# denix56/SI-Mamba

Measured on AMD Instinct MI355X. Metric: point-clouds/sec (fwd+bwd), higher is better.
Workload: dtype f32; 1 GPU; PointMamba classifier train step (FPS+kNN grouping, encoder, spectral SAST ordering, 12 Mamba blocks d=384 at L=1024, head, AdamW), 1024 pts -> 128 patches; global_batch=64, per_gpu_batch=64, npoints=1024, patches=128, mamba_seq_len=1024, parallelism=dp1, communicator_ranks=1, library_gemm=tuned solution table (si_mamba_amd/tuned/gemm_gfx950.csv)

## Files before the change

### include/simamba.h

```cpp
#ifndef SIMAMBA_H_
#define SIMAMBA_H_

#include <stddef.h>

#ifdef __cplusplus
extern "C" {
#endif

#define SIMAMBA_ABI_VERSION 9

#define SIMAMBA_F32  0
#define SIMAMBA_BF16 1

#define SIMAMBA_OK            0
#define SIMAMBA_E_NULLPTR    -1
#define SIMAMBA_E_SHAPE      -2
#define SIMAMBA_E_DTYPE      -3
#define SIMAMBA_E_DSTATE     -4
#define SIMAMBA_E_WIDTH      -5
#define SIMAMBA_E_WORKSPACE  -6
#define SIMAMBA_E_GROUPS     -7
#define SIMAMBA_E_ALIGN      -8
#define SIMAMBA_E_VARIANT    -9
#define SIMAMBA_E_BIAS       -10
// ... 107 lines not shown
                               int dim, int hidden_dtype, int out_dtype, void* stream);

#define SIMAMBA_NORM_RMS 1
int simamba_add_layer_norm_fwd_ex(const void* hidden, const float* residual, const float* rowscale,
                                  const float* weight, const float* bias, float* residual_out,
                                  void* normed, float* mean, float* rstd, int batch, int rows_per_batch,
                                  int dim, float eps, int hidden_dtype, int out_dtype, int flags, void* stream);
int simamba_add_layer_norm_bwd_ex(const void* dnormed, const float* dresidual_out,
                                  const float* residual_out, const float* mean, const float* rstd,
                                  const float* weight, const float* rowscale, float* dresidual,
                                  void* dhidden, float* dwb_partial, int batch, int rows_per_batch,
                                  int dim, int hidden_dtype, int out_dtype, int flags, void* stream);

int simamba_out_proj_add_ln_fwd(const void* y, const void* w, const float* residual, const float* rowscale,
                                const float* gamma, const float* beta, float* residual_out, void* normed, float* mean,
                                float* rstd, int batch, int K, int L, int C, float eps, int out_dtype, void* stream);
int simamba_out_proj_add_ln_fwd_ex(const void* y, const void* w, const float* residual, const float* rowscale,
                                   const float* gamma, const float* beta, float* residual_out, void* normed,
                                   float* mean, float* rstd, int batch, int K, int L, int C, float eps, int out_dtype,
                                   int flags, void* stream);

int simamba_in_proj_fwd(const void* x, const void* w, void* xz, int batch, int L, int C, int M, int io_dtype,
                        void* stream);

int simamba_bn_relu_grid(long long rows);
int simamba_bn_relu_fwd(const void* x, const float* gterm, int group, const float* weight, const float* bias,
                        float* running_mean, float* running_var, float momentum, float eps, int training,
                        void* y, float* mean, float* invstd, float* partial, long long rows, int C,
                        long long ld, int io_dtype, void* stream);
int simamba_bn_relu_bwd(const void* dy, const void* x, const float* gterm, int group, const float* weight,
                        const float* bias, const float* mean, const float* invstd, void* dx, float* dgterm,
                        int dgroup, float* dweight, float* dbias, float* partial, long long rows, int C,
                        long long ld, int io_dtype, int training, void* stream);
int simamba_bn_stats_local(const void* x, const float* gterm, int group, double* stats, long long stats_ld,
                           float* partial, long long rows, int C, long long ld, int io_dtype, void* stream);
int simamba_bn_stats_merge(const double* stats, int world, float* running_mean, float* running_var, float momentum,
                           float eps, float* mean, float* invstd, double* count, int C, void* stream);
int simamba_bn_relu_apply(const void* x, const float* gterm, int group, const float* weight, const float* bias,
                          const float* mean, const float* invstd, void* y, long long rows, int C, long long ld,
                          int io_dtype, void* stream);
int simamba_bn_relu_bwd_sums(const void* dy, const void* x, const float* gterm, int group, const float* weight,
                             const float* bias, const float* mean, const float* invstd, float* dweight,
                             float* dbias, float* partial, long long rows, int C, long long ld, int io_dtype,
                             void* stream);
int simamba_bn_relu_bwd_dx(const void* dy, const void* x, const float* gterm, int group, const float* weight,
                           const float* bias, const float* mean, const float* invstd, const float* sum_dweight,
                           const float* sum_dbias, const double* count, void* dx, float* dgterm, int dgroup,
                           long long rows, int C, long long ld, int io_dtype, void* stream);
int simamba_group_max_fwd(const void* x, void* out, unsigned char* idx, long long groups, int n, int C,
                          int io_dtype, void* stream);
int simamba_group_max_bwd(const void* dout, const unsigned char* idx, void* dx, long long groups, int n, int C,
                          int io_dtype, void* stream);

int simamba_three_nn(const float* xyz1, const float* xyz2, int* idx, float* weight, int batch, int N, int S,
                     void* stream);
int simamba_three_interpolate_fwd(const void* feats, const int* idx, const float* weight, void* out, int batch,
                                  int N, int S, int C, int io_dtype, void* stream);
int simamba_three_interpolate_bwd(const void* dout, const int* idx, const float* weight, float* dfeats, int batch,
                                  int N, int S, int C, int io_dtype, void* stream);

int simamba_chamfer_fwd(const float* pred, const float* gt, float* dist, unsigned char* idx1, unsigned char* idx2,
                        long long pairs, int n, int m, void* stream);
int simamba_chamfer_bwd(const float* pred, const float* gt, const float* ddist, const unsigned char* idx1,
                        const unsigned char* idx2, float* dpred, long long pairs, int n, int m, void* stream);

int simamba_knn_group(const float* points, const float* centers, long long* idx, int batch, int N, int G, int K,
                      void* stream);
int simamba_knn_group_ex(const float* points, const float* centers, const long long* len_points,
                         const long long* len_centers, long long* idx, int batch, int N, int G, int K, void* stream);

#define SIMAMBA_SPEC_SYMMETRIC   0x01u
#define SIMAMBA_SPEC_SELF_LOOP   0x02u
#define SIMAMBA_SPEC_BINARY      0x04u
#define SIMAMBA_SPEC_MATRIX_SYM  0x08u
#define SIMAMBA_SPEC_SMALLEST    0x10u
#define SIMAMBA_SPEC_SIGMA_MEAN  0x20u
#define SIMAMBA_SPEC_LARGE_G     0x40u

int simamba_knn_graph(const float* points, float* adj, void* workspace, size_t ws_bytes,
                      int B, int G, int F, int knn, float alpha, unsigned flags, void* stream);

int simamba_laplacian_topk(const float* adj, float* evals, float* evecs, long long* order,
                           float* all_evals, float* all_evecs, int B, int G, int k,
                           unsigned flags, void* stream);

size_t simamba_laplacian_topk_workspace_bytes(int B, int G);
int simamba_laplacian_topk_ex(const float* adj, float* evals, float* evecs, long long* order,
                              void* workspace, size_t ws_bytes, int B, int G, int k, unsigned flags,
                              void* stream);

size_t simamba_spectral_workspace_bytes(int B, int G);

int simamba_spectral_topk(const float* centers, float* evals, float* evecs, long long* order,
                          void* workspace, size_t ws_bytes, int B, int G, int knn, float alpha,
                          int k, unsigned flags, void* stream);

int simamba_farthest_point_sample(const float* points, long long* idx, float* centers, int B, int N,
                                  int K, void* stream);
int simamba_farthest_point_sample_ex(const float* points, const long long* lengths, const long long* start,
                                     long long* idx, float* centers, int B, int N, int K, void* stream);

int simamba_argsort_rows(const float* vals, long long* idx, int rows, int n, void* stream);

#ifdef __cplusplus
}
#endif
// ... 2 lines not shown
```

### si_mamba_amd/_lib.py

```python
from __future__ import annotations

import ctypes
import os
from ctypes import c_char_p, c_float, c_int, c_longlong, c_size_t, c_uint, c_void_p

_HERE = os.path.dirname(os.path.abspath(__file__))
LIB_PATH = os.path.join(_HERE, "libsimamba_hip.so")

F32, BF16 = 0, 1

SPEC_SYMMETRIC = 0x01
SPEC_SELF_LOOP = 0x02
SPEC_BINARY = 0x04
SPEC_MATRIX_SYM = 0x08
SPEC_SMALLEST = 0x10
SPEC_SIGMA_MEAN = 0x20
SPEC_LARGE_G = 0x40
SPEC_MAX_G = 128
SPEC_MAX_G_LARGE = 512

SCAN_AUTO, SCAN_ROWSCAN, SCAN_LPC2, SCAN_LPC4, SCAN_MIX = 0, 1, 2, 4, 6
CKPT_ROW, CKPT_SEQ = 128, 16
BWD_DETERMINISTIC = 1
NORM_RMS = 1
# ... 21 lines not shown
    "simamba_selective_scan_bwd_ex": (c_int, [_P, _P, _P, _P, _P, _P, _P, _P, _P, _P,
                                              _P, _P, _P, _P, _P, _P, _P, _P,
                                              c_int, c_int, c_int, c_int, c_int, c_int,
                                              _LL, _LL, _LL, _LL, _LL, c_int, c_int, _P, _LL, _P]),
    "simamba_selective_scan_dt_fwd": (c_int, [_P, _P, _P, _P, _P, _P, _P, _P, _P, _P,
                                              c_int, c_int, c_int, c_int, c_int, c_int,
                                              _LL, _LL, _LL, c_int, c_int, _P]),
    "simamba_selective_scan_dt_bwd": (c_int, [_P, _P, _P, _P, _P, _P, _P, _P, _P,
                                              _P, _P, _P, _P, _P, _P, _P, _P,
                                              c_int, c_int, c_int, c_int, c_int, c_int,
                                              _LL, _LL, _LL, _LL, _P]),
    "simamba_selective_scan_dt_bwd_ex": (c_int, [_P, _P, _P, _P, _P, _P, _P, _P, _P,
                                                 _P, _P, _P, _P, _P, _P, _P, _P,
                                                 c_int, c_int, c_int, c_int, c_int, c_int,
                                                 _LL, _LL, _LL, _LL, c_int, _P, _LL, _P]),
    "simamba_xdt_proj_fwd": (c_int, [_P, _P, _P, _P, _P, c_int, c_int, c_int, c_int, c_int, c_int, _LL, _P]),
    "simamba_conv_xdt_proj_fwd": (c_int, [_P, _P, _P, _P, _P, _P, _P, _P, c_int, c_int, c_int, c_int, c_int, c_int, _LL,
                                          _P]),
    "simamba_seq_gather_fwd": (c_int, [_P, _P, _P, c_int, c_int, c_int, c_int, _LL, c_int, _P]),
    "simamba_seq_gather_bwd": (c_int, [_P, _P, _P, c_int, c_int, c_int, c_int, c_int, _LL, c_int, _P]),
    "simamba_causal_conv1d_fwd": (c_int, [_P, _P, _P, _P, c_int, c_int, c_int, c_int, c_int, c_int, _LL, _P]),
    "simamba_causal_conv1d_bwd": (c_int, [_P, _P, _P, _P, _P, _P, _P,
                                          c_int, c_int, c_int, c_int, c_int, c_int, _LL, _LL, _P]),
    "simamba_causal_conv1d_bwd_workspace_floats": (_LL, [c_int, c_int, c_int, c_int, c_int]),
    "simamba_causal_conv1d_bwd_ex": (c_int, [_P, _P, _P, _P, _P, _P, _P,
                                             c_int, c_int, c_int, c_int, c_int, c_int, _LL, _LL, c_int, _P, _LL, _P]),
    "simamba_add_layer_norm_grid": (c_int, [c_int, c_int]),
    "simamba_add_layer_norm_fwd": (c_int, [_P, _P, _P, _P, _P, _P, _P, _P, _P, c_int, c_int, c_int, c_float,
                                           c_int, c_int, _P]),
    "simamba_add_layer_norm_bwd": (c_int, [_P, _P, _P, _P, _P, _P, _P, _P, _P, _P, c_int, c_int, c_int,
                                           c_int, c_int, _P]),
    "simamba_add_layer_norm_fwd_ex": (c_int, [_P, _P, _P, _P, _P, _P, _P, _P, _P, c_int, c_int, c_int, c_float,
                                              c_int, c_int, c_int, _P]),
    "simamba_add_layer_norm_bwd_ex": (c_int, [_P, _P, _P, _P, _P, _P, _P, _P, _P, _P, c_int, c_int, c_int,
                                              c_int, c_int, c_int, _P]),
    "simamba_out_proj_add_ln_fwd": (c_int, [_P, _P, _P, _P, _P, _P, _P, _P, _P, _P, c_int, c_int, c_int, c_int, c_float,
                                            c_int, _P]),
    "simamba_out_proj_add_ln_fwd_ex": (c_int, [_P, _P, _P, _P, _P, _P, _P, _P, _P, _P, c_int, c_int, c_int, c_int,
                                               c_float, c_int, c_int, _P]),
    "simamba_in_proj_fwd": (c_int, [_P, _P, _P, c_int, c_int, c_int, c_int, c_int, _P]),
    "simamba_bn_relu_grid": (c_int, [_LL]),
    "simamba_bn_relu_fwd": (c_int, [_P, _P, c_int, _P, _P, _P, _P, c_float, c_float, c_int, _P, _P, _P, _P, _LL, c_int,
                                    _LL, c_int, _P]),
    "simamba_bn_relu_bwd": (c_int, [_P, _P, _P, c_int, _P, _P, _P, _P, _P, _P, c_int, _P, _P, _P, _LL, c_int, _LL,
                                    c_int, c_int, _P]),
    "simamba_bn_stats_local": (c_int, [_P, _P, c_int, _P, _LL, _P, _LL, c_int, _LL, c_int, _P]),
    "simamba_bn_stats_merge": (c_int, [_P, c_int, _P, _P, c_float, c_float, _P, _P, _P, c_int, _P]),
    "simamba_bn_relu_apply": (c_int, [_P, _P, c_int, _P, _P, _P, _P, _P, _LL, c_int, _LL, c_int, _P]),
    "simamba_bn_relu_bwd_sums": (c_int, [_P, _P, _P, c_int, _P, _P, _P, _P, _P, _P, _P, _LL, c_int, _LL, c_int, _P]),
    "simamba_bn_relu_bwd_dx": (c_int, [_P, _P, _P, c_int, _P, _P, _P, _P, _P, _P, _P, _P, _P, c_int, _LL, c_int, _LL,
                                       c_int, _P]),
    "simamba_group_max_fwd": (c_int, [_P, _P, _P, _LL, c_int, c_int, c_int, _P]),
    "simamba_group_max_bwd": (c_int, [_P, _P, _P, _LL, c_int, c_int, c_int, _P]),
    "simamba_three_nn": (c_int, [_P, _P, _P, _P, c_int, c_int, c_int, _P]),
    "simamba_three_interpolate_fwd": (c_int, [_P, _P, _P, _P, c_int, c_int, c_int, c_int, c_int, _P]),
    "simamba_three_interpolate_bwd": (c_int, [_P, _P, _P, _P, c_int, c_int, c_int, c_int, c_int, _P]),
    "simamba_chamfer_fwd": (c_int, [_P, _P, _P, _P, _P, _LL, c_int, c_int, _P]),
    "simamba_chamfer_bwd": (c_int, [_P, _P, _P, _P, _P, _P, _LL, c_int, c_int, _P]),
    "simamba_knn_group": (c_int, [_P, _P, _P, c_int, c_int, c_int, c_int, _P]),
    "simamba_knn_group_ex": (c_int, [_P, _P, _P, _P, _P, c_int, c_int, c_int, c_int, _P]),
    "simamba_knn_graph": (c_int, [_P, _P, _P, c_size_t, c_int, c_int, c_int, c_int, c_float, c_uint, _P]),
    "simamba_laplacian_topk": (c_int, [_P, _P, _P, _P, _P, _P, c_int, c_int, c_int, c_uint, _P]),
    "simamba_laplacian_topk_workspace_bytes": (c_size_t, [c_int, c_int]),
    "simamba_laplacian_topk_ex": (c_int, [_P, _P, _P, _P, _P, c_size_t, c_int, c_int, c_int, c_uint, _P]),
    "simamba_spectral_workspace_bytes": (c_size_t, [c_int, c_int]),
    "simamba_spectral_topk": (c_int, [_P, _P, _P, _P, _P, c_size_t, c_int, c_int, c_int, c_float,
                                      c_int, c_uint, _P]),
    "simamba_argsort_rows": (c_int, [_P, _P, c_int, c_int, _P]),
    "simamba_farthest_point_sample": (c_int, [_P, _P, _P, c_int, c_int, c_int, _P]),
    "simamba_farthest_point_sample_ex": (c_int, [_P, _P, _P, _P, _P, c_int, c_int, c_int, _P]),
}

_lib = None


def load():
    global _lib
    if _lib is not None:
        return _lib
    if not os.path.exists(LIB_PATH):
        raise RuntimeError(
            f"{LIB_PATH} not found: build it with `python -c 'import __graft_entry__ as g; g.build()'` "
            "or `make -C si_mamba_amd/csrc`.  si_mamba_amd has no CPU / eager fallback.")
    lib = ctypes.CDLL(LIB_PATH)
    for name, (res, args) in SIGNATURES.items():
        fn = getattr(lib, name)
        fn.restype = res
        fn.argtypes = args
    got = lib.simamba_abi_version()
    if got != ABI_VERSION:
        raise RuntimeError(f"libsimamba_hip.so ABI version {got}, binding expects {ABI_VERSION}")
    _lib = lib
    return lib


def check(rc: int, what: str):
    if rc != 0:
        msg = load().simamba_strerror(rc).decode()
        raise RuntimeError(f"{what} failed (rc={rc}): {msg}")


def ptr(t):
    return None if t is None else t.data_ptr()


def dtype_code(dtype):
# ... 81 lines not shown

class scan_variant(_Override):
    cell, coerce = _scan_variant, int

    def __init__(self, variant):
        super().__init__(variant)


def current_scan_variant():
    return _scan_variant[0]


_scan_ckpt = [0]


class scan_ckpt(_Override):
    cell, coerce = _scan_ckpt, int

    def __init__(self, step):
        super().__init__(step)


_spectral_large_g = [False]


class spectral_large_g(_Override):
    cell = _spectral_large_g

    def __init__(self, on=True):
        super().__init__(on)


def spectral_large_g_forced():
    return _spectral_large_g[0]


_fuse_dt = [None]
counters = {}


def count(name):
    counters[name] = counters.get(name, 0) + 1


class scan_fuse_dt(_Override):
    cell, coerce = _fuse_dt, staticmethod(_tristate)


def fuse_dt_enabled(dtype):
    import torch
    return (dtype == torch.bfloat16) if _fuse_dt[0] is None else _fuse_dt[0]


_fuse_out_norm = [True]
_hand_in_proj = [None]


class fuse_out_norm(_Override):
    cell = _fuse_out_norm


def fuse_out_norm_enabled():
    return _fuse_out_norm[0]


class hand_in_proj(_Override):
    cell, coerce = _hand_in_proj, staticmethod(_tristate)


def in_proj_hand_enabled(workgroups, dtype=None):
    import torch
    if _hand_in_proj[0] is not None:
        return _hand_in_proj[0]
    return dtype != torch.float32 and workgroups >= IN_PROJ_MIN_WORKGROUPS


IN_PROJ_MIN_WORKGROUPS = 192


def scan_plan_step(batch, dim, seqlen, dstate, dtype, *, softplus=True, has_z=True, act_addr_or=0, a_addr=0,
                   b_addr=0, c_addr=0, z_bs=0, dz_bs=0, bc_strides=(0, 0, 0)):
    lib = load()
    code = dtype_code(dtype)
    step = _scan_ckpt[0] or lib.simamba_scan_ckpt_step(batch, dim, seqlen, dstate, code)
    if step == CKPT_SEQ and not lib.simamba_scan_seq_applicable(
            batch, dim, seqlen, dstate, code, int(bool(softplus)), int(bool(has_z)), act_addr_or, a_addr, b_addr,
            c_addr, z_bs, dz_bs, *bc_strides):
        step = CKPT_ROW
    if _scan_variant[0] == SCAN_ROWSCAN:
        step = CKPT_ROW
    return step


def mixer_scan_operands(xz_addr, a_addr, dim, seqlen, dt_rank, dstate, esz, xz_bs):
    S = dt_rank + 2 * dstate
    return dict(softplus=True, has_z=True, act_addr_or=xz_addr | (xz_addr + dim * seqlen * esz), a_addr=a_addr,
                b_addr=dt_rank * esz, c_addr=(dt_rank + dstate) * esz, z_bs=xz_bs, dz_bs=xz_bs,
                bc_strides=(seqlen * S, 1, S))


def scan_plan(batch, dim, seqlen, dstate, dtype, device, need_grad, **operands):
    import torch
    step = scan_plan_step(batch, dim, seqlen, dstate, dtype, **operands)
    count("scan_ckpt_seq" if step == CKPT_SEQ else "scan_ckpt_row")
    if not need_grad:
        return step, None
# ... 46 lines not shown
```

### si_mamba_amd/encoder_ops.py

```python
from __future__ import annotations

import torch
import torch.distributed as dist

from . import _lib


_BN_MAX_C = 1024
_BN_CHUNK = 256


_SPLITK = 64
_SPLITK_MIN_ROWS = 512


class TokenLinearFn(torch.autograd.Function):

    @staticmethod
    def forward(ctx, x, weight, bias):
        y = torch.nn.functional.linear(x, weight, bias)
        ctx.save_for_backward(x, weight)
        ctx.has_bias = bias is not None
        return y

    @staticmethod
    def backward(ctx, dy):
        x, weight = ctx.saved_tensors
        dy = dy.contiguous()
        io = dy.dtype
        rows, n_out = dy.shape
        dx = dw = db = None
        if ctx.needs_input_grad[0]:
            dx = (dy @ weight.to(io)).to(x.dtype)
        if ctx.needs_input_grad[1]:
            xc = x.to(io).contiguous()
            if rows % _SPLITK == 0 and rows // _SPLITK >= _SPLITK_MIN_ROWS:
                m = rows // _SPLITK
                a = dy.view(_SPLITK, m, n_out).transpose(1, 2)
                b = xc.view(_SPLITK, m, xc.shape[1])
                part = torch.bmm(a, b) if io == torch.float32 else torch.bmm(a, b, out_dtype=torch.float32)
                dw = part.sum(0).to(weight.dtype)
            else:
                dw = (dy.t() @ xc).to(weight.dtype)
        if ctx.has_bias and ctx.needs_input_grad[2]:
            db = dy.sum(0, dtype=torch.float32).to(weight.dtype)
        return dx, dw, db


def token_linear(x, weight, bias=None):
    if x.is_cuda and x.dim() == 2 and torch.is_grad_enabled() and (weight.requires_grad or x.requires_grad):
        return TokenLinearFn.apply(x, weight, bias)
    return torch.nn.functional.linear(x, weight, bias)


def _slices(C):
    return [(c0, min(c0 + _BN_MAX_C, C)) for c0 in range(0, C, _BN_MAX_C)]


def _off(t, elems):
    return None if t is None else t.data_ptr() + elems * t.element_size()


def _abi(name, *args):
    _lib.check(getattr(_lib.load(), name)(*args), name)


def _slice_of(g, c0, c1, C):
    return None if g is None else (g if (c0 == 0 and c1 == C) else g[:, c0:c1].contiguous())


def _bn_partial(lib, rows, C, dev):
    return torch.empty(lib.simamba_bn_relu_grid(rows), 2, min(C, _BN_MAX_C), device=dev, dtype=torch.float32)


def _bn_operands(x, gterm, weight, bias):
    xc = x.contiguous()
    g, w, b = (None if t is None else t.float().contiguous() for t in (gterm, weight, bias))
    mean = torch.empty(xc.shape[1], device=xc.device, dtype=torch.float32)
    return xc, g, w, b, torch.empty_like(xc), mean, torch.empty_like(mean)


def _dtypes(*tensors):
    return tuple(None if t is None else t.dtype for t in tensors)


def _bn_grads(dtypes, dx, dgt, dw, db):
    xdtype, gdtype, wdtype, bdtype = dtypes
    return (dx.to(xdtype), None if dgt is None else dgt.to(gdtype), None,
            None if wdtype is None else dw.to(wdtype), None if bdtype is None else db.to(bdtype),
            None, None, None, None, None)


def _bn_dgroup(g, group):
    dgroup = 0 if g is None else (group if _BN_CHUNK % group == 0 else _BN_CHUNK)
    if g is not None and dgroup == _BN_CHUNK and group % _BN_CHUNK != 0:
        raise ValueError("bn_relu_fn: group must divide 256 or be a multiple of it")
    return dgroup


# ... 148 lines not shown
def _bn_step(bn):
    training = bn.training or bn.running_mean is None
    momentum = bn.momentum
    if bn.training and bn.track_running_stats and bn.num_batches_tracked is not None:
        bn.num_batches_tracked.add_(1)
        if momentum is None:
            momentum = 1.0 / float(bn.num_batches_tracked)
    rm = bn.running_mean if (bn.track_running_stats and (bn.training or not training)) else None
    rv = bn.running_var if rm is not None else None
    return training, 0.0 if momentum is None else momentum, rm, rv


def _dist_up():
    return dist.is_available() and dist.is_initialized()


def _bn_relu_local(x, bn, gterm, group):
    training, momentum, rm, rv = _bn_step(bn)
    return BnReluFn.apply(x, gterm, group, bn.weight, bn.bias, rm, rv, momentum, bn.eps, training)


def sync_bn_relu_fn(x, bn, gterm=None, group=0, process_group=None):
    if not isinstance(bn, (torch.nn.BatchNorm1d, torch.nn.SyncBatchNorm)):
        raise TypeError(f"sync_bn_relu_fn: expected nn.SyncBatchNorm or nn.BatchNorm1d, got {type(bn).__name__}")
    if not bn.training:
        return _bn_relu_local(x, bn, gterm, group)
    if x.shape[0] < 1:
        raise ValueError(f"sync_bn_relu_fn: this rank holds {x.shape[0]} rows; every rank needs at least 1")
    if not _dist_up():
        raise RuntimeError("sync_bn_relu_fn: torch.distributed has no initialised process group")
    if x.is_cuda and torch.cuda.is_current_stream_capturing():
        raise RuntimeError(_CAPTURE_MSG)
    if process_group is None:
        process_group = getattr(bn, "process_group", None)
    _, momentum, rm, rv = _bn_step(bn)
    return SyncBnReluFn.apply(x, gterm, group, bn.weight, bn.bias, rm, rv, momentum, bn.eps, process_group)


def _sync_world(bn):
    return dist.get_world_size(bn.process_group) if _dist_up() else 1


def bn_relu_fn(x, bn: torch.nn.BatchNorm1d, gterm=None, group=0):
    if type(bn) is torch.nn.SyncBatchNorm:
        if bn.training and _sync_world(bn) > 1:
            return sync_bn_relu_fn(x, bn, gterm=gterm, group=group)
    elif type(bn) is not torch.nn.BatchNorm1d:
        if gterm is not None:
            x = x + gterm.to(x.dtype).repeat_interleave(group, dim=0)
        return torch.relu(bn(x))
    return _bn_relu_local(x, bn, gterm, group)


class GroupMaxFn(torch.autograd.Function):
    @staticmethod
    def forward(ctx, x):
        _lib.require_gpu(x, "group_max_fn")
        xc = x.contiguous()
        groups, n, C = xc.shape
        dev = xc.device
        code = _lib.dtype_code(xc.dtype)
        out = torch.empty(groups, C, device=dev, dtype=xc.dtype)
        idx = torch.empty(groups, C, device=dev, dtype=torch.uint8)
        with torch.cuda.device(dev):
            _abi("simamba_group_max_fwd", xc.data_ptr(), out.data_ptr(), idx.data_ptr(), groups, n, C, code,
                 _lib.stream_ptr(dev))
        ctx.save_for_backward(idx)
        ctx.meta = (groups, n, C, code, xc.dtype)
        return out

    @staticmethod
    def backward(ctx, dout):
        (idx,) = ctx.saved_tensors
        groups, n, C, code, dtype = ctx.meta
        d = dout.to(dtype).contiguous()
        dx = torch.empty(groups, n, C, device=d.device, dtype=dtype)
        with torch.cuda.device(d.device):
            _abi("simamba_group_max_bwd", d.data_ptr(), idx.data_ptr(), dx.data_ptr(), groups, n, C, code,
                 _lib.stream_ptr(d.device))
        return dx


def group_max_fn(x):
    return GroupMaxFn.apply(x)
```

### si_mamba_amd/point_mamba.py

```python
from __future__ import annotations

from types import SimpleNamespace

import torch
import torch.nn as nn

from . import grouping, spectral
from .block import MixerModel
from .add_norm import add_layer_norm_fn
from .encoder_ops import bn_relu_fn, group_max_fn, token_linear


class Group(nn.Module):

    def __init__(self, num_group, group_size):
        super().__init__()
        self.num_group = num_group
        self.group_size = group_size
        self.fps_fn = grouping.sample_farthest_points

    @torch.no_grad()
    def _indices(self, xyz, lengths=None):
        if lengths is not None:
            if not (xyz.is_cuda and xyz.shape[1] <= 8192):
                raise NotImplementedError("Group: lengths are taken by the HIP kernels only (a ROCm device, clouds of "
                                          "up to 8192 points)")
            need = max(self.num_group, self.group_size)
            if not torch.cuda.is_current_stream_capturing():
                shortest = int(lengths.min())
                if shortest < need:
                    raise ValueError(f"Group: the shortest cloud has {shortest} points, every cloud needs at least "
                                     f"{need} (max of num_group = {self.num_group} and group_size = {self.group_size})")
            center, _ = self.fps_fn(xyz, self.num_group, lengths=lengths)
            return center, grouping.knn_group(center, xyz, self.group_size, lengths=lengths)
        center, _ = self.fps_fn(xyz, self.num_group)
        if xyz.is_cuda and xyz.shape[1] <= 8192:
            return center, grouping.knn_group(center, xyz, self.group_size)
        d = torch.cdist(center, xyz)
        nn_idx = d.topk(self.group_size, dim=-1, largest=False, sorted=False)[1]
        return center, nn_idx

    def forward(self, xyz, *, lengths=None):
        B, N, _ = xyz.shape
        center, nn_idx = self._indices(xyz, lengths)
        flat = (nn_idx + torch.arange(B, device=xyz.device).view(-1, 1, 1) * N).view(-1)
        nb = xyz.reshape(B * N, -1)[flat].view(B, self.num_group, self.group_size, 3).contiguous()
        return nb - center.unsqueeze(2), center, nb


class Encoder(nn.Module):

    def __init__(self, encoder_channel):
        super().__init__()
        self.encoder_channel = encoder_channel
        self.fused = True
        self.first_conv = nn.Sequential(nn.Conv1d(3, 128, 1), nn.BatchNorm1d(128), nn.ReLU(inplace=True),
                                        nn.Conv1d(128, 256, 1))
        self.second_conv = nn.Sequential(nn.Conv1d(512, 512, 1), nn.BatchNorm1d(512), nn.ReLU(inplace=True),
                                         nn.Conv1d(512, self.encoder_channel, 1))

    def forward(self, point_groups):
        bs, g, n, _ = point_groups.shape
        c1, bn1, _, c2 = self.first_conv
        c3, bn2, _, c4 = self.second_conv
        lin = torch.nn.functional.linear
        x = point_groups.reshape(bs * g * n, 3)
        if self.fused and x.is_cuda and 256 % n == 0:
            lin = token_linear
            x = bn_relu_fn(lin(x, c1.weight.squeeze(-1), c1.bias), bn1)
            f = lin(x, c2.weight.squeeze(-1), c2.bias)
            cf = f.shape[1]
            fg = group_max_fn(f.view(bs * g, n, cf))
            w3 = c3.weight.squeeze(-1)
            gterm = lin(fg, w3[:, :cf], c3.bias)
            x = bn_relu_fn(lin(f, w3[:, cf:]), bn2, gterm=gterm, group=n)
            f = lin(x, c4.weight.squeeze(-1), c4.bias)
            return group_max_fn(f.view(bs * g, n, self.encoder_channel)).reshape(bs, g, self.encoder_channel)
        x = torch.relu(bn1(lin(x, c1.weight.squeeze(-1), c1.bias)))
        f = lin(x, c2.weight.squeeze(-1), c2.bias).view(bs * g, n, 256)
        fg = f.max(dim=1, keepdim=True)[0]
        x = torch.cat([fg.expand(-1, n, -1), f], dim=2).reshape(bs * g * n, 512)
        x = torch.relu(bn2(lin(x, c3.weight.squeeze(-1), c3.bias)))
        f = lin(x, c4.weight.squeeze(-1), c4.bias).view(bs * g, n, self.encoder_channel)
        return f.max(dim=1)[0].reshape(bs, g, self.encoder_channel)


def default_config(**over):
    cfg = dict(trans_dim=384, depth=12, cls_dim=15, group_size=32, num_group=128, encoder_dims=384,
               rms_norm=False, drop_path=0.1, drop_out=0., method="SAST", reverse=True, knn_graph=20,
               k_top_eigenvectors=4, alpha=10., smallest=True, symmetric=True, self_loop=False,
               binary=True, matrix="laplacian")
    cfg.update(over)
    return SimpleNamespace(**cfg)


def plackett_luce_dist(logits):
    return torch.sum(logits - torch.logcumsumexp(logits.flip(-1), dim=-1).flip(-1), dim=-1)


class PointMamba(nn.Module):
    def __init__(self, config, **kwargs):
        super().__init__()
        self.config = config
        self.trans_dim = config.trans_dim
        self.depth = config.depth
        self.cls_dim = config.cls_dim
        self.group_size = config.group_size
        self.num_group = config.num_group
        self.encoder_dims = config.encoder_dims
        self.group_divider = Group(num_group=self.num_group, group_size=self.group_size)
        self.encoder = Encoder(encoder_channel=self.encoder_dims)
        self.drop_path = getattr(config, "drop_path", 0.)
        self.rms_norm = getattr(config, "rms_norm", False)
        self.drop_out_in_block = getattr(config, "drop_out_in_block", 0.)
        self.pos_embed = nn.Sequential(nn.Linear(3, 128), nn.GELU(), nn.Linear(128, self.trans_dim))
        self.blocks = MixerModel(d_model=self.trans_dim, n_layer=self.depth, rms_norm=self.rms_norm,
                                 drop_out_in_block=self.drop_out_in_block, drop_path=self.drop_path)
        self.norm = nn.LayerNorm(self.trans_dim)
        self.cls_head_finetune = nn.Sequential(
            nn.Linear(self.trans_dim, 256), nn.BatchNorm1d(256), nn.ReLU(inplace=True), nn.Dropout(0.5),
            nn.Linear(256, 256), nn.BatchNorm1d(256), nn.ReLU(inplace=True), nn.Dropout(0.5),
            nn.Linear(256, self.cls_dim))
        self.loss_ce = nn.CrossEntropyLoss()
        self.drop_out = nn.Dropout(getattr(config, "drop_out", 0.))
        self.method = config.method
        self.reverse = config.reverse
        self.k_top_eigenvectors = config.k_top_eigenvectors
        self.smallest = config.smallest
        self.knn_graph = config.knn_graph
        self.symmetric = config.symmetric
# ... 104 lines not shown
```

Measured before the change: 1123 point-clouds/s.

## Fuse encoder linear+group-max backward using sparse argmax gradients

Adds HIP kernels that compute the backward of a linear layer followed by a per-group max directly from the sparse max indices. This avoids materialising the dense scattered gradient and running dense GEMMs on mostly-zero rows; only one of n rows per channel contributes. It also fuses the group-max backward with the residual add for the second conv's dual output. The cost is custom kernels with split-range partial sums plus a deterministic reduction, in place of tuned library GEMMs.

```diff
diff --git a/include/simamba.h b/include/simamba.h
--- a/include/simamba.h
+++ b/include/simamba.h
@@ -183,6 +183,15 @@
 int simamba_group_max_bwd(const void* dout, const unsigned char* idx, void* dx, long long groups, int n, int C,
                           int io_dtype, void* stream);
 
+long long simamba_linear_max_bwd_dw_workspace_floats(long long P, int n, int Cin, int Cout);
+int simamba_linear_max_bwd_dx(const void* g, const unsigned char* idx, const float* W, void* dX, long long P, int n,
+                              int Cin, int Cout, int io_dtype, void* stream);
+int simamba_linear_max_bwd_dw(const void* g, const unsigned char* idx, const void* X, float* dW, float* db,
+                              float* workspace, long long workspace_floats, long long P, int n, int Cin, int Cout,
+                              int io_dtype, void* stream);
+int simamba_group_max_bwd_add(const void* dout, const unsigned char* idx, const void* base, void* dx,
+                              long long groups, int n, int C, int io_dtype, void* stream);
+
 int simamba_three_nn(const float* xyz1, const float* xyz2, int* idx, float* weight, int batch, int N, int S,
                      void* stream);
 int simamba_three_interpolate_fwd(const void* feats, const int* idx, const float* weight, void* out, int batch,
diff --git a/si_mamba_amd/_lib.py b/si_mamba_amd/_lib.py
--- a/si_mamba_amd/_lib.py
+++ b/si_mamba_amd/_lib.py
@@ -97,6 +97,10 @@
                                        c_int, _P]),
     "simamba_group_max_fwd": (c_int, [_P, _P, _P, _LL, c_int, c_int, c_int, _P]),
     "simamba_group_max_bwd": (c_int, [_P, _P, _P, _LL, c_int, c_int, c_int, _P]),
+    "simamba_linear_max_bwd_dw_workspace_floats": (_LL, [_LL, c_int, c_int, c_int]),
+    "simamba_linear_max_bwd_dx": (c_int, [_P, _P, _P, _P, _LL, c_int, c_int, c_int, c_int, _P]),
+    "simamba_linear_max_bwd_dw": (c_int, [_P, _P, _P, _P, _P, _P, _LL, _LL, c_int, c_int, c_int, c_int, _P]),
+    "simamba_group_max_bwd_add": (c_int, [_P, _P, _P, _P, _LL, c_int, c_int, c_int, _P]),
     "simamba_three_nn": (c_int, [_P, _P, _P, _P, c_int, c_int, c_int, _P]),
     "simamba_three_interpolate_fwd": (c_int, [_P, _P, _P, _P, c_int, c_int, c_int, c_int, c_int, _P]),
     "simamba_three_interpolate_bwd": (c_int, [_P, _P, _P, _P, c_int, c_int, c_int, c_int, c_int, _P]),
@@ -284,6 +288,18 @@
     return (dtype == torch.bfloat16) if _fuse_dt[0] is None else _fuse_dt[0]
 
 
+_linear_max_sparse = [None]
+
+
+class linear_max_sparse(_Override):
+    cell, coerce = _linear_max_sparse, staticmethod(_tristate)
+
+
+def linear_max_sparse_enabled(dtype):
+    import torch
+    return (dtype == torch.float32) if _linear_max_sparse[0] is None else _linear_max_sparse[0]
+
+
 _fuse_out_norm = [True]
 _hand_in_proj = [None]
 
diff --git a/si_mamba_amd/csrc/linear_max.hip b/si_mamba_amd/csrc/linear_max.hip
--- /dev/null
+++ b/si_mamba_amd/csrc/linear_max.hip
@@ -0,0 +1,308 @@
+#include "det_reduce.h"
+#include "host_common.h"
+
+namespace simamba {
+
+constexpr int kLmMaxRows = 32;
+constexpr int kLmMaxCin = 512, kLmMaxCout = 512;
+constexpr int kDxThreads = 512;
+constexpr int kDxCols = 64;
+constexpr int kDwThreads = 256;
+constexpr int kDwCh = 96;
+constexpr int kDwMaxRanges = 128;
+
+__device__ __forceinline__ void xcd_map(int b, int S, int& s, int& q) {
+  const int x = b & 7, j = b >> 3;
+  s = j % S;
+  q = (j / S) * 8 + x;
+}
+
+static int round_up8(long long v) { return static_cast<int>((v + 7) / 8 * 8); }
+static int dx_ranges(long long P, int S) {
+  const long long cap = (256 + S - 1) / S, want = (P + 3) / 4;
+  return round_up8(want < cap ? want : cap);
+}
+static int dw_ranges(long long P) {
+  const long long want = (P + 15) / 16;
+  return round_up8(want < kDwMaxRanges ? want : kDwMaxRanges);
+}
+
+template <typename T>
+__global__ __launch_bounds__(kDxThreads) void linear_max_dx_kernel(
+    const T* __restrict__ g, const unsigned char* __restrict__ idx, const float* __restrict__ W, T* __restrict__ dX,
+    int P, int n, int Cin, int Cout, int S, int ppr) {
+  extern __shared__ __align__(16) unsigned char smem[];
+  float* Wl = reinterpret_cast<float*>(smem);
+  int2* ent = reinterpret_cast<int2*>(Wl + Cout * kDxCols);
+  int* cnt = reinterpret_cast<int*>(ent + Cout);
+  int* rowstart = cnt + 8 * kLmMaxRows;
+  int s, q;
+  xcd_map(blockIdx.x, S, s, q);
+  const int p0 = q * ppr, p1 = min(P, p0 + ppr);
+  if (p0 >= p1) return;
+  const int tid = threadIdx.x, lane = tid & 63, wave = tid >> 6;
+  const int col0 = s * kDxCols;
+  for (int e = tid; e < Cout * (kDxCols / 4); e += kDxThreads) {
+    const int c = e / (kDxCols / 4), j = e % (kDxCols / 4);
+    *reinterpret_cast<float4*>(Wl + c * kDxCols + 4 * j) =
+        *reinterpret_cast<const float4*>(W + static_cast<size_t>(c) * Cin + col0 + 4 * j);
+  }
+  const int nchunks = (Cout + 63) / 64;
+  const int c = wave * 64 + lane;
+  const bool valid = c < Cout;
+  const unsigned long long lt = (1ull << lane) - 1ull;
+  int idn = 255;
+  float gn = 0.f;
+  if (valid) {
+    idn = idx[static_cast<size_t>(p0) * Cout + c];
+    gn = to_f32<T>(g[static_cast<size_t>(p0) * Cout + c]);
+  }
+  const int h = tid >> 5, cp = tid & 31;
+  __syncthreads();
+  for (int p = p0; p < p1; ++p) {
+    const int idv = idn;
+    const float gv = gn;
+    if (valid && p + 1 < p1) {
+      idn = idx[static_cast<size_t>(p + 1) * Cout + c];
+      gn = to_f32<T>(g[static_cast<size_t>(p + 1) * Cout + c]);
+    }
+    int rank = 0, mycnt = 0;
+    for (int r = 0; r < n; ++r) {
+      const unsigned long long m = __ballot(idv == r);
+      if (idv == r) rank = __popcll(m & lt);
+      if (lane == r) mycnt = __popcll(m);
+    }
+    if (lane < kLmMaxRows) cnt[wave * kLmMaxRows + lane] = mycnt;
+    __syncthreads();
+    if (wave == 0) {
+      int run = 0;
+      if (lane < kLmMaxRows) {
+        for (int k = 0; k < nchunks; ++k) {
+          const int t = cnt[k * kLmMaxRows + lane];
+          cnt[k * kLmMaxRows + lane] = run;
+          run += t;
+        }
+      }
+      int incl = run;
+#pragma unroll
+      for (int d = 1; d < 64; d <<= 1) {
+        const int t = __shfl_up(incl, d);
+        if (lane >= d) incl += t;
+      }
+      if (lane <= kLmMaxRows) rowstart[lane] = incl - run;
+    }
+    __syncthreads();
+    if (idv < n)
+      ent[rowstart[idv] + cnt[wave * kLmMaxRows + idv] + rank] = make_int2(c * kDxCols * 4, __float_as_int(gv));
+    __syncthreads();
+    for (int r = h; r < n; r += kDxThreads / 32) {
+      const int beg = rowstart[r], end = rowstart[r + 1];
+      float a0 = 0.f, a1 = 0.f;
+      for (int i = beg; i < end; i += 4) {
+        int2 e[4];
+        float2 w[4];
+#pragma unroll
+        for (int u = 0; u < 4; ++u) e[u] = ent[min(i + u, end - 1)];
+#pragma unroll
+        for (int u = 0; u < 4; ++u)
+          w[u] = *reinterpret_cast<const float2*>(reinterpret_cast<const unsigned char*>(Wl) + e[u].x + cp * 8);
+#pragma unroll
+        for (int u = 0; u < 4; ++u) {
+          const float gg = (i + u < end) ? __int_as_float(e[u].y) : 0.f;
+          a0 = fmaf(gg, w[u].x, a0);
+          a1 = fmaf(gg, w[u].y, a1);
+        }
+      }
+      Pack<T, 2> o;
+      o.v[0] = from_f32<T>(a0);
+      o.v[1] = from_f32<T>(a1);
+      *reinterpret_cast<Pack<T, 2>*>(dX + (static_cast<size_t>(p) * n + r) * Cin + col0 + 2 * cp) = o;
+    }
+  }
+}
+
+template <typename T>
+__global__ __launch_bounds__(kDwThreads, 2) void linear_max_dw_kernel(
+    const T* __restrict__ g, const unsigned char* __restrict__ idx, const T* __restrict__ X, float* __restrict__ part,
+    float* __restrict__ dbpart, int P, int n, int Cin, int Cout, int S, int ppr) {
+  extern __shared__ __align__(16) unsigned char smem[];
+  const int xbytes = n * Cin * static_cast<int>(sizeof(T));
+  int4* meta = reinterpret_cast<int4*>(smem + xbytes);
+  int s, q;
+  xcd_map(blockIdx.x, S, s, q);
+  const int p0 = min(P, q * ppr), p1 = min(P, p0 + ppr);
+  const int c0 = s * kDwCh, tid = threadIdx.x;
+  const bool act = 2 * tid < Cin;
+  const int col = act ? 2 * tid : 0;
+  const bool mine = tid < kDwCh && c0 + tid < Cout;
+  const unsigned char* xcol = smem + col * sizeof(T);
+  float acc[kDwCh][2];
+#pragma unroll
+  for (int c = 0; c < kDwCh; ++c) acc[c][0] = acc[c][1] = 0.f;
+  float dbacc = 0.f;
+  const int nvec = xbytes / 16;
+  for (int p = p0; p < p1; ++p) {
+    __syncthreads();
+    const uint4* __restrict__ src = reinterpret_cast<const uint4*>(X + static_cast<size_t>(p) * n * Cin);
+#pragma unroll 8
+    for (int v = tid; v < nvec; v += kDwThreads) reinterpret_cast<uint4*>(smem)[v] = src[v];
+    if (tid < kDwCh) {
+      int row = 0;
+      float gg = 0.f;
+      if (mine) {
+        row = idx[static_cast<size_t>(p) * Cout + c0 + tid];
+        gg = to_f32<T>(g[static_cast<size_t>(p) * Cout + c0 + tid]);
+        dbacc += gg;
+      }
+      gg = row < n ? gg : 0.f;
+      row = min(row, n - 1);
+      reinterpret_cast<int2*>(meta)[tid] = make_int2(row * Cin * static_cast<int>(sizeof(T)), __float_as_int(gg));
+    }
+    __syncthreads();
+#pragma unroll
+    for (int c = 0; c < kDwCh; c += 2) {
+      const int4 m = meta[c / 2];
+      const Pack<T, 2> x0 = *reinterpret_cast<const Pack<T, 2>*>(xcol + m.x);
+      const Pack<T, 2> x1 = *reinterpret_cast<const Pack<T, 2>*>(xcol + m.z);
+      const float g0 = __int_as_float(m.y), g1 = __int_as_float(m.w);
+      acc[c][0] = fmaf(g0, to_f32<T>(x0.v[0]), acc[c][0]);
+      acc[c][1] = fmaf(g0, to_f32<T>(x0.v[1]), acc[c][1]);
+      acc[c + 1][0] = fmaf(g1, to_f32<T>(x1.v[0]), acc[c + 1][0]);
+      acc[c + 1][1] = fmaf(g1, to_f32<T>(x1.v[1]), acc[c + 1][1]);
+      if ((c & 15) == 14) __builtin_amdgcn_sched_barrier(0);
+    }
+  }
+  if (act) {
+#pragma unroll
+    for (int c = 0; c < kDwCh; ++c) {
+      if (c0 + c < Cout)
+        *reinterpret_cast<float2*>(part + (static_cast<size_t>(q) * Cout + c0 + c) * Cin + col) =
+            make_float2(acc[c][0], acc[c][1]);
+    }
+  }
+  if (mine) dbpart[static_cast<size_t>(q) * Cout + c0 + tid] = dbacc;
+}
+
+template <typename T>
+__global__ void group_max_bwd_add_kernel(const T* __restrict__ dout, const unsigned char* __restrict__ idx,
+                                         const T* base, T* dx, long long groups, int n, int C) {
+  const long long e = static_cast<long long>(blockIdx.x) * blockDim.x + threadIdx.x;
+  const int cq = C / 4;
+  if (e >= groups * cq) return;
+  const long long g = e / cq;
+  const int c = static_cast<int>(e - g * cq) * 4;
+  const Pack<T, 4> d = *reinterpret_cast<const Pack<T, 4>*>(dout + g * C + c);
+  const uchar4 id4 = *reinterpret_cast<const uchar4*>(idx + g * C + c);
+  const int id[4] = {id4.x, id4.y, id4.z, id4.w};
+  if (!base) {
+#pragma unroll
+    for (int i = 0; i < 4; ++i) {
+      if (id[i] < n) {
+        T* q = dx + (g * n + id[i]) * C + c + i;
+        *q = from_f32<T>(to_f32<T>(*q) + to_f32<T>(d.v[i]));
+      }
+    }
+    return;
+  }
+#pragma unroll 4
+  for (int r = 0; r < n; ++r) {
+    const long long o = (g * n + r) * C + c;
+    Pack<T, 4> v = *reinterpret_cast<const Pack<T, 4>*>(base + o);
+#pragma unroll
+    for (int i = 0; i < 4; ++i)
+      if (id[i] == r) v.v[i] = from_f32<T>(to_f32<T>(v.v[i]) + to_f32<T>(d.v[i]));
+    *reinterpret_cast<Pack<T, 4>*>(dx + o) = v;
+  }
+}
+
+constexpr int kNothingToDo = 1;
+static int entry_result(int rc) { return rc == kNothingToDo ? SIMAMBA_OK : rc; }
+
+static int lm_check(int io_dtype, long long P, int n, int Cin, int Cout) {
+  if (const int rc = check_io_dtype(io_dtype)) return rc;
+  if (P == 0) return kNothingToDo;
+  if (P < 0 || P > (1ll << 24) || n < 1 || n > kLmMaxRows) return SIMAMBA_E_SHAPE;
+  if (Cin < kDxCols || Cin > kLmMaxCin || (Cin % kDxCols) != 0) return SIMAMBA_E_SHAPE;
+  if (Cout < 4 || Cout > kLmMaxCout || (Cout % 4) != 0) return SIMAMBA_E_SHAPE;
+  return SIMAMBA_OK;
+}
+
+template <typename K>
+static int lds_cap(K kernel, size_t bytes) {
+  if (bytes <= 64 * 1024) return 0;
+  return static_cast<int>(hipFuncSetAttribute(reinterpret_cast<const void*>(kernel),
+                                              hipFuncAttributeMaxDynamicSharedMemorySize, static_cast<int>(bytes)));
+}
+
+}
+
+using namespace simamba;
+
+extern "C" long long simamba_linear_max_bwd_dw_workspace_floats(long long P, int n, int Cin, int Cout) {
+  const int rc = lm_check(SIMAMBA_F32, P, n, Cin, Cout);
+  if (rc) return rc == kNothingToDo ? 0 : rc;
+  return static_cast<long long>(dw_ranges(P)) * (static_cast<long long>(Cout) * Cin + Cout);
+}
+
+extern "C" int simamba_linear_max_bwd_dx(const void* g, const unsigned char* idx, const float* W, void* dX,
+                                         long long P, int n, int Cin, int Cout, int io_dtype, void* stream) {
+  if (const int rc = lm_check(io_dtype, P, n, Cin, Cout)) return entry_result(rc);
+  if (!g || !idx || !W || !dX) return SIMAMBA_E_NULLPTR;
+  if (!aligned16(W) || !aligned16(dX)) return SIMAMBA_E_ALIGN;
+  const int S = Cin / kDxCols, Q = dx_ranges(P, S);
+  const int ppr = static_cast<int>((P + Q - 1) / Q);
+  const size_t lds = static_cast<size_t>(Cout) * (kDxCols * 4 + 8) + sizeof(int) * (8 * kLmMaxRows + kLmMaxRows + 4);
+  int rc = SIMAMBA_OK;
+  with_io_type(io_dtype, [&](auto tag) {
+    using T = decltype(tag);
+    if ((rc = lds_cap(linear_max_dx_kernel<T>, lds))) return;
+    hipLaunchKernelGGL(linear_max_dx_kernel<T>, dim3(S * Q), dim3(kDxThreads), lds, static_cast<hipStream_t>(stream),
+                       static_cast<const T*>(g), idx, W, static_cast<T*>(dX), static_cast<int>(P), n, Cin, Cout, S,
+                       ppr);
+  });
+  return rc ? rc : static_cast<int>(hipGetLastError());
+}
+
+extern "C" int simamba_linear_max_bwd_dw(const void* g, const unsigned char* idx, const void* X, float* dW, float* db,
+                                         float* workspace, long long workspace_floats, long long P, int n, int Cin,
+                                         int Cout, int io_dtype, void* stream) {
+  if (const int rc = lm_check(io_dtype, P, n, Cin, Cout)) return entry_result(rc);
+  if (!g || !idx || !X || !dW) return SIMAMBA_E_NULLPTR;
+  const int S = (Cout + kDwCh - 1) / kDwCh, Q = dw_ranges(P);
+  const long long per = static_cast<long long>(Cout) * Cin;
+  if (!workspace || workspace_floats < Q * (per + Cout)) return SIMAMBA_E_WORKSPACE;
+  if (!aligned16(X) || !aligned16(workspace) || !aligned16(dW)) return SIMAMBA_E_ALIGN;
+  const int ppr = static_cast<int>((P + Q - 1) / Q);
+  const size_t lds = static_cast<size_t>(n) * Cin * io_esz(io_dtype) + sizeof(int2) * kDwCh;
+  hipStream_t s = static_cast<hipStream_t>(stream);
+  float* dbpart = workspace + Q * per;
+  int rc = SIMAMBA_OK;
+  with_io_type(io_dtype, [&](auto tag) {
+    using T = decltype(tag);
+    if ((rc = lds_cap(linear_max_dw_kernel<T>, lds))) return;
+    hipLaunchKernelGGL(linear_max_dw_kernel<T>, dim3(S * Q), dim3(kDwThreads), lds, s, static_cast<const T*>(g), idx,
+                       static_cast<const T*>(X), workspace, dbpart, static_cast<int>(P), n, Cin, Cout, S, ppr);
+  });
+  if (rc) return rc;
+  const DetSumJob jobs[2] = {{workspace, dW, per, per, Q}, {dbpart, db, Cout, db ? Cout : 0, Q}};
+  if (const int e = det_sum_launch(jobs, 2, s)) return e;
+  return static_cast<int>(hipGetLastError());
+}
+
+extern "C" int simamba_group_max_bwd_add(const void* dout, const unsigned char* idx, const void* base, void* dx,
+                                         long long groups, int n, int C, int io_dtype, void* stream) {
+  if (const int rc = check_io_dtype(io_dtype)) return rc;
+  if (groups == 0) return SIMAMBA_OK;
+  if (groups < 0 || n < 1 || n > 256 || C < 4 || (C % 4) != 0) return SIMAMBA_E_SHAPE;
+  if (!dout || !idx || !dx) return SIMAMBA_E_NULLPTR;
+  const long long total = groups * (C / 4);
+  if (total > 0x7fffffffll * 256) return SIMAMBA_E_SHAPE;
+  if (base == dx) base = nullptr;
+  with_io_type(io_dtype, [&](auto tag) {
+    using T = decltype(tag);
+    hipLaunchKernelGGL(group_max_bwd_add_kernel<T>, dim3(static_cast<unsigned>((total + 255) / 256)), dim3(256), 0,
+                       static_cast<hipStream_t>(stream), static_cast<const T*>(dout), idx, static_cast<const T*>(base),
+                       static_cast<T*>(dx), groups, n, C);
+  });
+  return static_cast<int>(hipGetLastError());
+}
diff --git a/si_mamba_amd/encoder_ops.py b/si_mamba_amd/encoder_ops.py
--- a/si_mamba_amd/encoder_ops.py
+++ b/si_mamba_amd/encoder_ops.py
@@ -26,25 +26,29 @@
     @staticmethod
     def backward(ctx, dy):
         x, weight = ctx.saved_tensors
-        dy = dy.contiguous()
-        io = dy.dtype
-        rows, n_out = dy.shape
-        dx = dw = db = None
-        if ctx.needs_input_grad[0]:
-            dx = (dy @ weight.to(io)).to(x.dtype)
-        if ctx.needs_input_grad[1]:
-            xc = x.to(io).contiguous()
-            if rows % _SPLITK == 0 and rows // _SPLITK >= _SPLITK_MIN_ROWS:
-                m = rows // _SPLITK
-                a = dy.view(_SPLITK, m, n_out).transpose(1, 2)
-                b = xc.view(_SPLITK, m, xc.shape[1])
-                part = torch.bmm(a, b) if io == torch.float32 else torch.bmm(a, b, out_dtype=torch.float32)
-                dw = part.sum(0).to(weight.dtype)
-            else:
-                dw = (dy.t() @ xc).to(weight.dtype)
-        if ctx.has_bias and ctx.needs_input_grad[2]:
-            db = dy.sum(0, dtype=torch.float32).to(weight.dtype)
-        return dx, dw, db
+        return _token_linear_grads(x, weight, dy, ctx.has_bias, ctx.needs_input_grad)
+
+
+def _token_linear_grads(x, weight, dy, has_bias, needs):
+    dy = dy.contiguous()
+    io = dy.dtype
+    rows, n_out = dy.shape
+    dx = dw = db = None
+    if needs[0]:
+        dx = (dy @ weight.to(io)).to(x.dtype)
+    if needs[1]:
+        xc = x.to(io).contiguous()
+        if rows % _SPLITK == 0 and rows // _SPLITK >= _SPLITK_MIN_ROWS:
+            m = rows // _SPLITK
+            a = dy.view(_SPLITK, m, n_out).transpose(1, 2)
+            b = xc.view(_SPLITK, m, xc.shape[1])
+            part = torch.bmm(a, b) if io == torch.float32 else torch.bmm(a, b, out_dtype=torch.float32)
+            dw = part.sum(0).to(weight.dtype)
+        else:
+            dw = (dy.t() @ xc).to(weight.dtype)
+    if has_bias and needs[2]:
+        db = dy.sum(0, dtype=torch.float32).to(weight.dtype)
+    return dx, dw, db
 
 
 def token_linear(x, weight, bias=None):
@@ -299,34 +303,148 @@
     return _bn_relu_local(x, bn, gterm, group)
 
 
+def _group_max_fwd(x):
+    _lib.require_gpu(x, "group_max_fn")
+    xc = x.contiguous()
+    groups, n, C = xc.shape
+    dev = xc.device
+    out = torch.empty(groups, C, device=dev, dtype=xc.dtype)
+    idx = torch.empty(groups, C, device=dev, dtype=torch.uint8)
+    with torch.cuda.device(dev):
+        _abi("simamba_group_max_fwd", xc.data_ptr(), out.data_ptr(), idx.data_ptr(), groups, n, C,
+             _lib.dtype_code(xc.dtype), _lib.stream_ptr(dev))
+    return out, idx
+
+
+def _group_max_bwd(d, idx, n, base=None):
+    groups, C = d.shape
+    dx = torch.empty(groups, n, C, device=d.device, dtype=d.dtype)
+    code, st = _lib.dtype_code(d.dtype), _lib.stream_ptr(d.device)
+    with torch.cuda.device(d.device):
+        if base is None:
+            _abi("simamba_group_max_bwd", d.data_ptr(), idx.data_ptr(), dx.data_ptr(), groups, n, C, code, st)
+        else:
+            _abi("simamba_group_max_bwd_add", d.data_ptr(), idx.data_ptr(), base.data_ptr(), dx.data_ptr(), groups, n, C,
+                 code, st)
+    return dx
+
+
 class GroupMaxFn(torch.autograd.Function):
     @staticmethod
     def forward(ctx, x):
-        _lib.require_gpu(x, "group_max_fn")
-        xc = x.contiguous()
-        groups, n, C = xc.shape
-        dev = xc.device
-        code = _lib.dtype_code(xc.dtype)
-        out = torch.empty(groups, C, device=dev, dtype=xc.dtype)
-        idx = torch.empty(groups, C, device=dev, dtype=torch.uint8)
-        with torch.cuda.device(dev):
-            _abi("simamba_group_max_fwd", xc.data_ptr(), out.data_ptr(), idx.data_ptr(), groups, n, C, code,
-                 _lib.stream_ptr(dev))
+        out, idx = _group_max_fwd(x)
         ctx.save_for_backward(idx)
-        ctx.meta = (groups, n, C, code, xc.dtype)
+        ctx.meta = (x.shape[1], x.dtype)
         return out
 
     @staticmethod
     def backward(ctx, dout):
         (idx,) = ctx.saved_tensors
-        groups, n, C, code, dtype = ctx.meta
-        d = dout.to(dtype).contiguous()
-        dx = torch.empty(groups, n, C, device=d.device, dtype=dtype)
-        with torch.cuda.device(d.device):
-            _abi("simamba_group_max_bwd", d.data_ptr(), idx.data_ptr(), dx.data_ptr(), groups, n, C, code,
-                 _lib.stream_ptr(d.device))
-        return dx
+        n, dtype = ctx.meta
+        return _group_max_bwd(dout.to(dtype).contiguous(), idx, n)
 
 
 def group_max_fn(x):
     return GroupMaxFn.apply(x)
+
+
+def _linear_max_sparse_ok(x, weight, g, n):
+    if not (x.is_cuda and x.dtype == g.dtype and g.dtype in (torch.float32, torch.bfloat16)):
+        return False
+    if not _lib.linear_max_sparse_enabled(g.dtype):
+        return False
+    return _lib.load().simamba_linear_max_bwd_dw_workspace_floats(g.shape[0], n, x.shape[1], g.shape[1]) > 0
+
+
+def _linear_max_sparse_grads(x, weight, g, idx, n, has_bias, needs):
+    P, n_out = g.shape
+    n_in = x.shape[1]
+    dev = x.device
+    xc = x.contiguous()
+    code, st = _lib.dtype_code(g.dtype), _lib.stream_ptr(dev)
+    dx = dw = db = None
+    with torch.cuda.device(dev), _lib.timed("linear_max_bwd", dev):
+        if needs[0]:
+            dx = torch.empty_like(xc)
+            _abi("simamba_linear_max_bwd_dx", g.data_ptr(), idx.data_ptr(), weight.float().contiguous().data_ptr(),
+                 dx.data_ptr(), P, n, n_in, n_out, code, st)
+        if needs[1] or (has_bias and needs[2]):
+            floats = _lib.load().simamba_linear_max_bwd_dw_workspace_floats(P, n, n_in, n_out)
+            ws = torch.empty(floats, device=dev, dtype=torch.float32)
+            dw = torch.empty(n_out, n_in, device=dev, dtype=torch.float32)
+            db = torch.empty(n_out, device=dev, dtype=torch.float32) if has_bias else None
+            _abi("simamba_linear_max_bwd_dw", g.data_ptr(), idx.data_ptr(), xc.data_ptr(), dw.data_ptr(), _lib.ptr(db),
+                 ws.data_ptr(), floats, P, n, n_in, n_out, code, st)
+            dw = dw.to(weight.dtype)
+            db = None if db is None else db.to(weight.dtype)
+    return dx, dw, db
+
+
+class LinearGroupMaxFn(torch.autograd.Function):
+
+    @staticmethod
+    def forward(ctx, x, weight, bias, n):
+        f = torch.nn.functional.linear(x, weight, bias)
+        out, idx = _group_max_fwd(f.view(f.shape[0] // n, n, f.shape[1]))
+        ctx.save_for_backward(x, weight, idx)
+        ctx.meta = (int(n), f.dtype, bias is not None)
+        return out
+
+    @staticmethod
+    def backward(ctx, dout):
+        x, weight, idx = ctx.saved_tensors
+        n, dtype, has_bias = ctx.meta
+        g = dout.to(dtype).contiguous()
+        if _linear_max_sparse_ok(x, weight, g, n):
+            _lib.count("linear_max_sparse")
+            grads = _linear_max_sparse_grads(x, weight, g, idx, n, has_bias, ctx.needs_input_grad)
+        else:
+            _lib.count("linear_max_dense")
+            dy = _group_max_bwd(g, idx, n).view(-1, g.shape[1])
+            grads = _token_linear_grads(x, weight, dy, has_bias, ctx.needs_input_grad)
+        return (*grads, None)
+
+
+def _wants_grad(x, weight):
+    return x.is_cuda and x.dim() == 2 and torch.is_grad_enabled() and (weight.requires_grad or x.requires_grad)
+
+
+def linear_group_max(x, weight, bias, n):
+    if _wants_grad(x, weight):
+        return LinearGroupMaxFn.apply(x, weight, bias, n)
+    f = torch.nn.functional.linear(x, weight, bias)
+    f = f.view(f.shape[0] // n, n, f.shape[1])
+    return group_max_fn(f) if f.is_cuda else f.max(dim=1)[0]
+
+
+class TokenLinearMaxFn(torch.autograd.Function):
+
+    @staticmethod
+    def forward(ctx, x, weight, bias, n):
+        f = torch.nn.functional.linear(x, weight, bias)
+        fg, idx = _group_max_fwd(f.view(f.shape[0] // n, n, f.shape[1]))
+        ctx.save_for_backward(x, weight, idx)
+        ctx.meta = (int(n), f.dtype, bias is not None)
+        ctx.set_materialize_grads(False)
+        return f, fg
+
+    @staticmethod
+    def backward(ctx, df, dfg):
+        x, weight, idx = ctx.saved_tensors
+        n, dtype, has_bias = ctx.meta
+        if df is None and dfg is None:
+            return None, None, None, None
+        if dfg is None:
+            dy = df.to(dtype)
+        else:
+            base = None if df is None else df.to(dtype).contiguous().view(-1, n, df.shape[1])
+            dy = _group_max_bwd(dfg.to(dtype).contiguous(), idx, n, base=base).view(-1, dfg.shape[1])
+        return (*_token_linear_grads(x, weight, dy, has_bias, ctx.needs_input_grad), None)
+
+
+def token_linear_max(x, weight, bias, n):
+    if _wants_grad(x, weight):
+        return TokenLinearMaxFn.apply(x, weight, bias, n)
+    f = torch.nn.functional.linear(x, weight, bias)
+    f3 = f.view(f.shape[0] // n, n, f.shape[1])
+    return f, (group_max_fn(f3) if f.is_cuda else f3.max(dim=1)[0])
diff --git a/si_mamba_amd/point_mamba.py b/si_mamba_amd/point_mamba.py
--- a/si_mamba_amd/point_mamba.py
+++ b/si_mamba_amd/point_mamba.py
@@ -8,7 +8,7 @@
 from . import grouping, spectral
 from .block import MixerModel
 from .add_norm import add_layer_norm_fn
-from .encoder_ops import bn_relu_fn, group_max_fn, token_linear
+from .encoder_ops import bn_relu_fn, linear_group_max, token_linear, token_linear_max
 
 
 class Group(nn.Module):
@@ -68,14 +68,12 @@
         if self.fused and x.is_cuda and 256 % n == 0:
             lin = token_linear
             x = bn_relu_fn(lin(x, c1.weight.squeeze(-1), c1.bias), bn1)
-            f = lin(x, c2.weight.squeeze(-1), c2.bias)
+            f, fg = token_linear_max(x, c2.weight.squeeze(-1), c2.bias, n)
             cf = f.shape[1]
-            fg = group_max_fn(f.view(bs * g, n, cf))
             w3 = c3.weight.squeeze(-1)
             gterm = lin(fg, w3[:, :cf], c3.bias)
             x = bn_relu_fn(lin(f, w3[:, cf:]), bn2, gterm=gterm, group=n)
-            f = lin(x, c4.weight.squeeze(-1), c4.bias)
-            return group_max_fn(f.view(bs * g, n, self.encoder_channel)).reshape(bs, g, self.encoder_channel)
+            return linear_group_max(x, c4.weight.squeeze(-1), c4.bias, n).reshape(bs, g, self.encoder_channel)
         x = torch.relu(bn1(lin(x, c1.weight.squeeze(-1), c1.bias)))
         f = lin(x, c2.weight.squeeze(-1), c2.bias).view(bs * g, n, 256)
         fg = f.max(dim=1, keepdim=True)[0]
```

Measured after the change: 1122 point-clouds/s. About the same (-0.1%).
